# Blosc/c-blosc

Measured on NVIDIA H100. Metric: compress+decompress GB/s, higher is better.
Workload: dtype u8

## Files before the change

### c-blosc_b200/csrc/backend_cuda.cu

```cuda
#include <cuda_runtime.h>
#include <stdio.h>
#include <stdlib.h>

#include "b2_backend.h"
#include "dev_chunk.cuh"
#include "dev_filters.cuh"

struct b2_stream_s {
  cudaStream_t s;
};

#define B2_MAX_DEVICES 64
static int g_sms[B2_MAX_DEVICES];
static int g_prof_on = 0;
static double g_prof_ms[B2_K_COUNT];
static long long g_prof_n[B2_K_COUNT];
static long long g_launches = 0;

#define CK(call)                                                                              \
  do {                                                                                        \
    cudaError_t e_ = (call);                                                                  \
    if (e_ != cudaSuccess) {                                                                  \
      fprintf(stderr, "blosc_b200: CUDA error %s at %s:%d\n", cudaGetErrorString(e_), __FILE__, __LINE__); \
      return -1;                                                                              \
// ... 118 lines not shown
static void prof_resolve() {
  std::lock_guard<std::mutex> lk(g_prof_mu);
  for (auto& p : g_pending) {
    float ms = 0;
    cudaEventSynchronize(p.e1);
    cudaEventElapsedTime(&ms, p.e0, p.e1);
    g_prof_ms[p.kind] += ms; g_prof_n[p.kind]++;
    cudaEventDestroy(p.e0); cudaEventDestroy(p.e1);
  }
  g_pending.clear();
}

extern "C" void b2_prof_enable(int on) { g_prof_on = on; }
extern "C" void b2_prof_reset(void) { prof_resolve(); for (int i = 0; i < B2_K_COUNT; i++) { g_prof_ms[i] = 0; g_prof_n[i] = 0; } }
extern "C" int b2_prof_get(int kind, double* ms, long long* n) {
  if (kind < 0 || kind >= B2_K_COUNT) return -1;
  prof_resolve();
  if (ms) *ms = g_prof_ms[kind];
  if (n) *n = g_prof_n[kind];
  return 0;
}
extern "C" long long b2_launch_count(void) { return g_launches; }

extern "C" int b2_launch_filter(const FilterArgs* a, b2_stream_t s) {
  const bool bit = a->mode >= FILT_BITSHUFFLE;
  const bool inverse = a->mode == FILT_UNSHUFFLE || a->mode == FILT_BITUNSHUFFLE;
  const long long nblocks = (a->nbytes + a->blocksize - 1) / a->blocksize;
  const long long ipb = (a->blocksize / a->typesize + FILT_TILE - 1) / FILT_TILE + 1;
  long long ctas = (nblocks * ipb + FILT_WARPS - 1) / FILT_WARPS;
  void (*kern)(FilterArgs) = a->typesize == 2 ? filter_kernel<2> : a->typesize == 4 ? filter_kernel<4> : a->typesize == 8 ? filter_kernel<8> : filter_kernel<0>;
  const size_t smem = bit ? FILT_WARPS * 16 * FILT_TILE : 0;
  int per_sm = 0;
  if (cudaOccupancyMaxActiveBlocksPerMultiprocessor(&per_sm, kern, FILT_WARPS * 32, smem) != cudaSuccess || per_sm < 1) { cudaGetLastError(); per_sm = 4; }
  const long long cap = (long long)num_sms() * per_sm;
  if (ctas > cap) ctas = cap;
  if (ctas < 1) ctas = 1;
  ProfScope ps(inverse ? B2_K_UNFILTER : B2_K_FILTER, s->s);
  kern<<<(unsigned)ctas, FILT_WARPS * 32, smem, s->s>>>(*a);
  CK(cudaGetLastError());
  return 0;
}

static int team_wanted(const EncodeArgs* a) {
  static int env = -2;
  if (env == -2) { const char* e = getenv("BLOSC_B200_LZ4_TEAM"); env = (e && *e) ? (atoi(e) != 0) : -1; }
  if (a->codec != B2_CODEC_LZ4 || a->table_bytes != LZ4_TABLE_BYTES) return 0;
  return env >= 0 ? env : (a->map.nsplits == 4 && !a->many);
}

#ifdef B2_LZ4_CYCLES
extern "C" int b2_lz4_cycles_read(unsigned long long* dst, int nstreams) {
  if (nstreams > LZ4C_MAXSTREAMS) nstreams = LZ4C_MAXSTREAMS;
  CK(cudaDeviceSynchronize());
  CK(cudaMemcpyFromSymbol(dst, g_lz4_cycles, (size_t)nstreams * LZ4C_N * sizeof(unsigned long long)));
  return nstreams;
}
#endif

template <class Args>
static Args take_tickets(const Args* a, long long jobs, long long drawers) {
  Args args = *a;
  args.queue_base = *a->queue_base_host;
  *a->queue_base_host += (unsigned)jobs + (unsigned)drawers;
  return args;
}

extern "C" int b2_launch_encode(const EncodeArgs* a, b2_stream_t s) {
  if (team_wanted(a)) {
    int ctas = a->map.nstreams;
    const int cap = num_sms() * TEAM_CTAS_PER_SM;
    if (ctas > cap) ctas = cap;
    if (ctas <= 0) return 0;
    ProfScope ps(B2_K_ENCODE, s->s);
    EncodeArgs args = take_tickets(a, a->map.nstreams, ctas);
    args.num_sms = num_sms();
    encode_team_kernel<<<ctas, TEAM_WARPS * 32, TEAM_SMEM_BYTES, s->s>>>(args);
    CK(cudaGetLastError());
    return 0;
  }
  int wpc = 65536 / a->table_bytes;
  if (wpc > 4) wpc = 4;
  if (wpc < 1) wpc = 1;
  const int ctas = (a->map.nstreams + wpc - 1) / wpc;
  if (ctas <= 0) return 0;
  ProfScope ps(B2_K_ENCODE, s->s);
  encode_kernel<<<ctas, wpc * 32, (size_t)wpc * a->table_bytes, s->s>>>(take_tickets(a, a->map.nstreams, ctas * wpc));
  CK(cudaGetLastError());
  return 0;
}

extern "C" int b2_launch_fast(const FastArgs* a, b2_stream_t s) {
  if (a->map.nstreams <= 0) return 0;
  {
    int ctas = (a->map.nstreams + INDEX_WARPS - 1) / INDEX_WARPS;
    ProfScope ps(B2_K_INDEX, s->s);
    index_kernel<<<ctas, INDEX_WARPS * 32, INDEX_WARPS * FAST_TAB_BYTES, s->s>>>(*a);
    CK(cudaGetLastError());
  }
  {
    void (*parse)(FastArgs) = a->codec == B2_CODEC_LZ4 ? parse_kernel : a->codec == B2_CODEC_ZLIB ? dparse_kernel : zparse_kernel;
    const long long njobs = (long long)a->map.nfull * a->map.nsplits * a->groups_full + a->groups_left;
    const int threads = a->threads;
    const size_t smem = (size_t)a->win_bytes + 64;
    int per_sm = (int)((size_t)220 * 1024 / (smem + 1024));
    if (per_sm * threads > 2048) per_sm = 2048 / threads;
    if (per_sm < 1) per_sm = 1;
    long long ctas = njobs;
// ... 108 lines not shown
```

### c-blosc_b200/csrc/dev_chunk.cuh

```cuda
#pragma once
#include "b2_args.h"
#include "dev_blosclz.cuh"
#include "dev_common.cuh"
#include "dev_inflate.cuh"
#include "dev_lz4.cuh"
#include "dev_lz4fast.cuh"
#include "dev_lz4dpair.cuh"
#include "dev_zstd.cuh"
#include "dev_zstdenc.cuh"
#include "dev_deflate.cuh"
#include "dev_snappy.cuh"



DEV int next_stream(int* queue, unsigned base, const StreamMap& m) {
  int job = 0;
  if (lane_id() == 0) job = (int)((unsigned)atomicAdd(queue, 1) - base);
  job = __shfl_sync(FULLMASK, job, 0);
  if (job >= m.nstreams) return -1;
  const int nfs = m.nfull * m.nsplits;
  if (m.leftover) {
    if (job == 0) return nfs;
    job--;
  }
// ... 112 lines not shown
    if (lane_id() == 0) { a.csizes[idx] = c; a.needs[idx] = need; }
    mine++;
    __syncwarp();
  }
  return mine;
}

__global__ void encode_kernel(EncodeArgs a) {
#ifdef SIMT_EMU
  u8* smem = simt::g_dynsmem;
#else
  extern __shared__ __align__(16) u8 smem[];
#endif
  const int warp = (int)(threadIdx.x >> 5);
  void* tab = smem + (size_t)warp * a.table_bytes;
  const int mine = encode_streams(a, [&](int, const u8* in, int len, u8* out, int* need) {
    if (a.codec == B2_CODEC_LZ4) {
      if (a.table_bytes == LZ4_TAB17_BYTES) return lz4_encode_warp<false, true>(in, len, out, len, a.accel, tab, need);
      if (len < 65536 + LZ4_MFLIMIT - 1) return lz4_encode_warp<true>(in, len, out, len, a.accel, tab, need);
      return lz4_encode_warp<false>(in, len, out, len, a.accel, tab, need);
    }
    return blz_encode_warp(a.clevel, in, len, out, len, a.split_flag, tab, a.table_bytes, need);
  });
  streams_done(a.done, a.map.nstreams, mine, [&] { if (a.fold_scan) warp_scan_blocks(a.scan); });
}


#define TEAM_WARPS 4
#define TEAM_CTAS_PER_SM 8
#define TEAM_SMEM_BYTES (LZ4_TABLE_BYTES + ((LZ4T_SMEM_BYTES + 15) & ~15))
#define TEAM_SM_SLOTS 1024
#ifndef SIMT_EMU
__device__ unsigned g_team_sm_seq[TEAM_SM_SLOTS];
#endif
__global__ void __launch_bounds__(TEAM_WARPS * 32, TEAM_CTAS_PER_SM) encode_team_kernel(EncodeArgs a) {
#ifdef SIMT_EMU
  u8* smem = simt::g_dynsmem;
#else
  extern __shared__ __align__(16) u8 smem[];
#endif
  void* tab = smem;
  Lz4Team* tm = (Lz4Team*)(smem + LZ4_TABLE_BYTES);
  const int warp = (int)(threadIdx.x >> 5);
  int walker = (int)((blockIdx.x / (unsigned)(a.num_sms > 0 ? a.num_sms : 1)) & 3u);
#ifndef SIMT_EMU
  if (lane_id() == 0) { unsigned w; asm volatile("mov.u32 %0, %%warpid;" : "=r"(w)); tm->sub[warp] = (int)(w & 3u); }
  if (threadIdx.x == 0) {
    unsigned sm; asm volatile("mov.u32 %0, %%smid;" : "=r"(sm));
    tm->slot = (int)(atomicAdd(&g_team_sm_seq[sm % TEAM_SM_SLOTS], 1u) & 3u);
  }
#endif
  if (threadIdx.x == 0) { tm->cmd = 0; tm->gen = 0; }
#ifdef B2_LZ4_CYCLES
  if (threadIdx.x < LZ4C_N) tm->cyc[threadIdx.x] = 0;
#endif
  __syncthreads();
#ifndef SIMT_EMU
  for (int k = 3; k >= 0; k--) if (tm->sub[k] == tm->slot) walker = k;
#endif
  if (warp != walker) { lz4_team_preparer(tm, tab, (warp - walker - 1) & 3); return; }
  const int mine = encode_streams(a, [&](int idx, const u8* in, int len, u8* out, int* need) {
    LZ4C_T(c_total);
    const int c = len < 65536 + LZ4_MFLIMIT - 1 ? lz4_encode_warp<true, false, true>(in, len, out, len, a.accel, tab, need, tm)
                                                 : lz4_encode_warp<false, false, true>(in, len, out, len, a.accel, tab, need, tm);
#ifdef B2_LZ4_CYCLES
    {
      const unsigned long long total = (unsigned long long)(clock64() - c_total);
      unsigned smid, wid;
      asm volatile("mov.u32 %0, %%smid;" : "=r"(smid));
      asm volatile("mov.u32 %0, %%warpid;" : "=r"(wid));
      __syncwarp();
      const int k = lane_id();
      if (idx < LZ4C_MAXSTREAMS && k < LZ4C_N)
        g_lz4_cycles[idx][k] = k == LZ4C_TOTAL ? total : k == LZ4C_SMID ? smid : k == LZ4C_SUBP ? (wid & 3u) : tm->cyc[k];
      __syncwarp();
      if (k < LZ4C_N) tm->cyc[k] = 0;
    }
#endif
    return c;
  });
  if (lane_id() == 0) *(volatile int*)&tm->cmd = LZ4T_QUIT;
  __syncwarp();
  __threadfence_block();
  bar_arrive(LZ4T_BAR_GO(0), 64); bar_arrive(LZ4T_BAR_GO(1), 64); bar_arrive(LZ4T_BAR_GO(2), 64);
  streams_done(a.done, a.map.nstreams, mine, [&] { if (a.fold_scan) warp_scan_blocks(a.scan); });
}


#define INDEX_WARPS 4
__global__ void __launch_bounds__(INDEX_WARPS * 32) index_kernel(FastArgs a) {
#ifdef SIMT_EMU
  u8* smem = simt::g_dynsmem;
#else
  extern __shared__ __align__(16) u8 smem[];
#endif
  const int warp = (int)(threadIdx.x >> 5);
  u32* tab = (u32*)(smem + (size_t)warp * FAST_TAB_BYTES);
  for (int idx = (int)blockIdx.x * INDEX_WARPS + warp; idx < a.map.nstreams; idx += (int)gridDim.x * INDEX_WARPS) {
    int block, len, split;
    long long off;
    stream_locate(a.map, idx, &block, &off, &len, &split);
    lz4f_index_warp(a.in + off, len, a.prev + off, tab, (u32)a.hash_mask);
    __syncwarp();
  }
}

template <bool ZSTD, int MAXD = 65535>
DEV void fast_parse_body(const FastArgs& a, u8* smem) {
  u32* sdata = (u32*)smem;
  int* sjob = (int*)(smem + a.win_bytes + 48);
  const int tid = (int)threadIdx.x, lane = lane_id();
  const int nfs = a.map.nfull * a.map.nsplits;
  const int njobs = nfs * a.groups_full + a.groups_left;
  const int spw = a.win_bytes / FAST_SEG;
  for (;;) {
    if (tid == 0) { sjob[0] = (int)((unsigned)atomicAdd(a.queue, 1) - a.queue_base); sjob[1] = 0; }
    __syncthreads();
    const int job = sjob[0];
    if (job >= njobs) break;
    int idx, g, K;
    if (job < a.groups_left) { idx = nfs; g = job; K = a.segs_left; }
    else {
      const int j = job - a.groups_left;
      const int per_split = a.map.nfull * a.groups_full;
      const int s = j / per_split, r = j - s * per_split;
      const int b = r / a.groups_full;
      g = r - b * a.groups_full;
      idx = b * a.map.nsplits + s; K = a.segs_full;
    }
// ... 612 lines not shown
```

### c-blosc_b200/csrc/dev_lz4.cuh

```cuda
#pragma once
#include "dev_common.cuh"

#define LZ4_MFLIMIT 12
#define LZ4_LASTLITERALS 5
#define LZ4_TABLE_BYTES 16384
#define LZ4_TAB17_BYTES (8192 + 512)
#define LZ4_TAB17_MINLEN 65547
#define LZ4_TAB17_MAXLEN 131072

template <bool U16>
DEV u32 lz4_hash_at(const u8* __restrict__ s, int pos) {
  if (U16) return (ld_u32(s + pos) * 2654435761u) >> (32 - 13);
  const u64 seq = (u64)ld_u32(s + pos) | ((u64)s[pos + 4] << 32);
  return (u32)(((seq << 24) * 889523592379ull) >> (64 - 12));
}

#define LZ4_SCALAR_PROBES 4

DEV long long lz4_probe_offset(int it, int accel) {
  if (it == 0) return 0;
  const long long m = it - 1;
  const long long c = m >> 6;
  return 1 + m * accel + 32 * c * (c - 1) + c * (m - 64 * c);
}
// ... 104 lines not shown
#else
  const int q = p + sb.sal;
  const u32* w = sb.s32 + (q >> 2);
  return __funnelshift_r(__ldg(w), __ldg(w + 1), (u32)(q & 3) * 8u);
#endif
}

template <bool U16>
DEV u32 lz4_hash_seq(u32 lo, u32 b4) {
  if (U16) return (lo * 2654435761u) >> (32 - 13);
  const u64 seq = (u64)lo | ((u64)(b4 & 0xffu) << 32);
  return (u32)(((seq << 24) * 889523592379ull) >> (64 - 12));
}

DEV int lz4_count_tail(const StreamBase& sb, const u8* __restrict__ s, int p, int q, int limit, int n) {
  if (p + 136 <= n) {
    const int lane = lane_id();
    const u32 x = ldp_win4(sb, p + 4 * lane) ^ ldp_win4(sb, q + 4 * lane);
    const unsigned full = __ballot_sync(FULLMASK, x == 0u);
    if (full != FULLMASK) {
      const int fl = __ffs((int)~full) - 1;
      return fl * 4 + eq_bytes32(__shfl_sync(FULLMASK, x, fl));
    }
    return 128 + warp_count_match(s, p + 128, q + 128, limit);
  }
  return warp_count_match(s, p, q, limit);
}

DEV int lz4_catch_up(const u8* __restrict__ s, int ip, int match, int anchor, int back) {
  const int lane = lane_id();
  for (;;) {
    const int a = ip - 1 - back - lane, b = match - 1 - back - lane;
    const bool ok = a >= anchor && b >= 0 && s[a] == s[b];
    const unsigned m = __ballot_sync(FULLMASK, ok);
    const int step = m == FULLMASK ? 32 : __ffs((int)~m) - 1;
    back += step;
    if (step < 32) return back;
  }
}

#ifdef SIMT_EMU
static long long g_dbg_lz4t_sessions = 0, g_dbg_lz4t_seqs = 0, g_dbg_lz4t_stale = 0, g_dbg_lz4t_x[6];
enum {
  LZ4T_S_HIT0,
  LZ4T_S_STALE = 4,
  LZ4T_S_MISS4,
  LZ4T_S_LIT,
  LZ4T_S_CAPPED,
  LZ4T_S_LONG,
  LZ4T_S_HUGE,
  LZ4T_S_N
};
static long long g_dbg_lz4t_s[LZ4T_S_N];
#define LZ4T_DBG(x) do { if (lane_id() == 0) (x)++; } while (0)
#else
#define LZ4T_DBG(x) do {} while (0)
#endif
#ifndef LZ4T_TILES
#define LZ4T_TILES 12
#endif
#ifndef LZ4T_AHEAD
#define LZ4T_AHEAD 8
#endif
#ifndef LZ4T_NAP
#define LZ4T_NAP 128
#endif
#define LZ4T_RING (32 * LZ4T_TILES)
#define LZ4T_BAR_IDLE(i) (1 + (i))
#define LZ4T_BAR_GO(i) (4 + (i))
#define LZ4T_QUIT 1
#define LZ4T_STOP 0x7fffffff
#define LZ4T_END 0xffffffffu
#define LZ4T_LONG 13
#define LZ4T_HSHIFT 19
#define LZ4T_BACKCAP 7
static_assert(LZ4T_TILES % 3 == 0 && LZ4T_AHEAD >= 1 && LZ4T_AHEAD < LZ4T_TILES && LZ4T_RING > 15 + 255 + 4, "team ring layout");
#define LZ4T_PREFETCH 512

enum {
  LZ4C_TOTAL,
  LZ4C_START,
  LZ4C_SESSION,
  LZ4C_FULLWAIT,
  LZ4C_REPROBE,
  LZ4C_SEARCH,
  LZ4C_SESSIONS, LZ4C_SEQS, LZ4C_CHAIN_SEQS,
  LZ4C_PREP_BUSY,
  LZ4C_PREP_OWN,
  LZ4C_PREP_GATHER,
  LZ4C_PREP_TILES,
  LZ4C_SMID, LZ4C_SUBP,
  LZ4C_STALE,
  LZ4C_N = 16
};
#ifdef B2_LZ4_CYCLES
#define LZ4C_MAXSTREAMS 16384
__device__ unsigned long long g_lz4_cycles[LZ4C_MAXSTREAMS][LZ4C_N];
#define LZ4C_T(t) const long long t = clock64()
#define LZ4C_TW(t) const long long t = TEAM ? clock64() : 0ll
#define LZ4C_ADD(k, v) do { if (lane_id() == 0) atomicAdd(&tm->cyc[k], (unsigned long long)(v)); } while (0)
#define LZ4C_SPAN(k, t) LZ4C_ADD(k, clock64() - (t))
#else
#define LZ4C_T(t) do {} while (0)
#define LZ4C_TW(t) do {} while (0)
#define LZ4C_ADD(k, v) do {} while (0)
#define LZ4C_SPAN(k, t) do {} while (0)
#endif

struct Lz4Team {
  uint2 vd[LZ4T_RING];
  int rdy[LZ4T_TILES];
  const u8* s;
  int n;
  int u16;
  int wt;
  int gen;
  int cmd;
  int sub[4];
  int slot;
#ifdef B2_LZ4_CYCLES
  unsigned long long cyc[LZ4C_N];
#endif
};
#define LZ4T_SMEM_BYTES ((int)sizeof(Lz4Team))

DEV int lz4t_ld_i32(const int* p) { return *(const volatile int*)p; }
DEV void lz4t_st_i32(int* p, int v) { *(volatile int*)p = v; }

template <bool U16>
DEV void lz4_team_prepare_tile(Lz4Team* tm, const void* tabmem, const u8* s, int n, int tile) {
  const int lane = lane_id();
  const int w0 = 32 * tile, p = w0 + lane;
  const int e = (tile % LZ4T_TILES) * 32 + lane;
  if (w0 + 31 + 24 > n) { tm->vd[e] = make_uint2(0u, LZ4T_END); return; }
  const StreamBase sb = make_stream_base(s);
  u32 r[5], a0, a1, a2, a3, a4, c0, c1, c2, c3, c4;
  LZ4C_T(c_t0);
  ldp_raw20(sb, p, r);
  ldp_take17(sb, p, r, a0, a1, a2, a3, a4);
  const u32 h = lz4_hash_seq<U16>(a0, a1);
  const int snap = U16 ? (int)((const volatile u16*)tabmem)[h] : (int)((const volatile u32*)tabmem)[h];
  u32 vx = h << LZ4T_HSHIFT, sn = LZ4T_END;
  if ((unsigned)snap < (unsigned)p) {
    LZ4C_T(c_t1);
    LZ4C_ADD(LZ4C_PREP_OWN, c_t1 - c_t0);
    ldp_gather17(sb, snap, c0, c1, c2, c3, c4);
    const u32 x1 = a1 ^ c1, x2 = a2 ^ c2, x3 = a3 ^ c3;
    u32 m;
    if (x1) m = (u32)(__ffs((int)x1) - 1) >> 3;
    else if (x2) m = 4u + ((u32)(__ffs((int)x2) - 1) >> 3);
    else if (x3) m = 8u + ((u32)(__ffs((int)x3) - 1) >> 3);
    else m = a4 != c4 ? 12u : (u32)LZ4T_LONG;
    const bool hit = (U16 || snap + 65535 >= p) && c0 == a0;
    u32 bk = 0;
    if (hit) {
      if (snap >= 8) {
        u32 p0, p1, q0, q1;
        ldp_win8(sb, p - 8, p0, p1);
        ldp_win8(sb, snap - 8, q0, q1);
        const u32 y1 = p1 ^ q1, z0 = (u32)__clz((int)(p0 ^ q0)) >> 3;
        bk = y1 ? (u32)__clz((int)y1) >> 3 : 4u + (z0 < 3u ? z0 : 3u);
      } else {
        while (bk < (u32)snap && s[p - 1 - (int)bk] == s[snap - 1 - (int)bk]) bk++;
      }
    }
    vx |= (hit ? 1u : 0u) | (m << 2) | (bk << 8);
    sn = (u32)snap;
    LZ4C_SPAN(LZ4C_PREP_GATHER, c_t1);
  }
  tm->vd[e] = make_uint2(vx, sn);
}

DEV void lz4_team_preparer(Lz4Team* tm, const void* tabmem, int i) {
  for (;;) {
    bar_sync(LZ4T_BAR_GO(i), 64);
    if (lz4t_ld_i32(&tm->cmd) == LZ4T_QUIT) return;
    const u8* s = *(const u8* const volatile*)&tm->s;
    const int n = lz4t_ld_i32(&tm->n), u16 = lz4t_ld_i32(&tm->u16);
    for (int tile = i;; tile += 3) {
      int w;
      for (;;) {
        w = __shfl_sync(FULLMASK, lz4t_ld_i32(&tm->wt), 0);
        if (w == LZ4T_STOP) break;
        if (tile < w) tile = w + (i + 3 - w % 3) % 3;
        if (tile <= w + LZ4T_AHEAD) break;
        __nanosleep(LZ4T_NAP);
      }
      if (w == LZ4T_STOP) break;
      LZ4C_T(c_go);
      lz4d_prefetch(s, 32 * tile + LZ4T_PREFETCH + lane_id(), n);
      if (u16) lz4_team_prepare_tile<true>(tm, tabmem, s, n, tile);
      else lz4_team_prepare_tile<false>(tm, tabmem, s, n, tile);
      __syncwarp();
      if (lane_id() == 0) { __threadfence_block(); lz4t_st_i32(&tm->rdy[tile % LZ4T_TILES], tile + 1); }
      LZ4C_SPAN(LZ4C_PREP_BUSY, c_go);
      LZ4C_ADD(LZ4C_PREP_TILES, 1);
    }
    __syncwarp();
    bar_arrive(LZ4T_BAR_IDLE(i), 64);
  }
}

DEV void lz4t_reach(Lz4Team* tm, int ip, int& wt, int& vt) {
  const int lo = (ip - 2) >> 5, hi = ip >> 5;
  if (lo > wt + LZ4T_AHEAD) LZ4T_DBG(g_dbg_lz4t_x[2]);
  if (lo != wt) { wt = lo; lz4t_st_i32(&tm->wt, lo); }
  for (int t = vt + 1 > lo ? vt + 1 : lo; t <= hi; t++) {
    const int* r = &tm->rdy[t % LZ4T_TILES];
    if (lz4t_ld_i32(r) != t + 1) {
      LZ4T_DBG(g_dbg_lz4t_x[5]);
      do { __syncwarp(); } while (__any_sync(FULLMASK, lz4t_ld_i32(r) != t + 1));
    }
  }
  if (hi > vt) vt = hi;
}

template <bool U16>
DEV bool lz4t_search(Lz4Team* tm, smem_addr_t vda, void* tabmem, const StreamBase& sb, int n, int anchor, int accel,
                     int& twt, int& tvt, u32& pk, u32& snap, int& ip, bool& hit, int& match, int& back, int& lit,
                     bool& have_mc, int& mc_carry) {
  u16* tab16 = (u16*)tabmem;
  u32* tab32 = (u32*)tabmem;
  const int mfl1 = n - LZ4_MFLIMIT + 1;
  ip = anchor + 1;
  int it = 0, pos = ip;
  for (;; it++) {
    if (it == LZ4_SCALAR_PROBES) { LZ4T_DBG(g_dbg_lz4t_s[LZ4T_S_MISS4]); lit = it; return false; }
    pos = ip + (it ? 1 + (it - 1) * accel : 0);
    if (ip + 1 + it * accel > mfl1) { lit = it; return false; }
    if ((pos >> 5) > tvt) lz4t_reach(tm, pos, twt, tvt);
    u32 qk, qs;
    smem_ld_u32x2(vda, ((u32)pos % (u32)LZ4T_RING) << 3, qk, qs);
    const u32 h = qk >> LZ4T_HSHIFT;
    const int cand = U16 ? (int)tab16[h] : (int)tab32[h];
    __syncwarp();
    if (cand != (int)qs) { LZ4T_DBG(g_dbg_lz4t_s[LZ4T_S_STALE]); lit = it; return false; }
    if (U16) tab16[h] = (u16)pos; else tab32[h] = (u32)pos;
    if (qk & 1u) { pk = qk; snap = qs; break; }
  }
  LZ4T_DBG(g_dbg_lz4t_s[LZ4T_S_HIT0 + it]);
  const int vb = (int)((pk >> 8) & 7u), dist = pos - anchor;
  const int bq = vb < dist ? vb : dist;
  int m = (int)((pk >> 2) & 15u);
  if (m == LZ4T_LONG) {
    LZ4T_DBG(g_dbg_lz4t_s[LZ4T_S_LONG]);
    m = LZ4T_LONG + lz4_count_tail(sb, sb.s, pos + 4 + LZ4T_LONG, (int)snap + 4 + LZ4T_LONG, n - LZ4_LASTLITERALS, n);
  }
  if (bq == dist && bq + m < 15 + 255) {
    const int mc = bq + m;
    snap -= (u32)bq;
    pk = 1u | ((u32)(mc < LZ4T_LONG ? mc : LZ4T_LONG) << 2);
    ip = anchor;
    LZ4C_ADD(LZ4C_SEQS, 1);
    LZ4C_ADD(LZ4C_CHAIN_SEQS, ~0ull);
    return true;
  }
  hit = true; ip = pos; match = (int)snap;
  have_mc = true; mc_carry = m;
  back = bq;
  if (vb == LZ4T_BACKCAP && dist > LZ4T_BACKCAP) {
    LZ4T_DBG(g_dbg_lz4t_s[LZ4T_S_CAPPED]);
    back = lz4_catch_up(sb.s, pos, (int)snap, anchor, LZ4T_BACKCAP);
  } else if (bq != dist) LZ4T_DBG(g_dbg_lz4t_s[LZ4T_S_LIT]);
  else LZ4T_DBG(g_dbg_lz4t_s[LZ4T_S_HUGE]);
  lit = pos - back - anchor;
  return false;
}

template <bool U16, bool PACK, bool TEAM>
DEV int lz4_encode_stream(const u8* __restrict__ s, const int n, u8* __restrict__ d, const int cap,
                          const int accel, void* tabmem, int* need_out, Lz4Team* tm) {
  const int lane = lane_id();
  const StreamBase sb = make_stream_base(s);
  u16* tab16 = (u16*)tabmem;
  u32* tab32 = (u32*)tabmem;
  u32* tabhi = (u32*)((u8*)tabmem + 8192);
#define LZ4_TGET(h) (U16 ? (int)tab16[h] : PACK ? ((int)tab16[h] | (int)(((tabhi[(h) >> 5] >> ((h) & 31u)) & 1u) << 16)) : (int)tab32[h])
#define LZ4_TPUT(h, v) do { if (U16) tab16[h] = (u16)(v); else if (PACK) { tab16[h] = (u16)(v); const u32 m_ = 1u << ((h) & 31u); \
                            if ((v) & 0x10000) atomicOr(&tabhi[(h) >> 5], m_); else atomicAnd(&tabhi[(h) >> 5], ~m_); } \
                            else tab32[h] = (u32)(v); } while (0)

  for (int i = lane; i < (PACK ? LZ4_TAB17_BYTES : LZ4_TABLE_BYTES) / 4; i += 32) tab32[i] = 0;
  __syncwarp();

  const bool limited = (long long)cap < (long long)n + n / 255 + 16;
  const int olimit = cap;
  const int mfl1 = n - LZ4_MFLIMIT + 1;
  const int matchlimit = n - LZ4_LASTLITERALS;
  int ip = 1, anchor = 0, op = 0;
  int need = 0;
#define LZ4_LIMIT(v) do { const int v_ = (v); if (v_ > need) need = v_; if (limited && v_ > olimit) return 0; } while (0)

  int w0 = -(1 << 30);
  u32 wq0 = 0, wq1 = 0, wq2 = 0, wh = 0;
  int pb = -(1 << 30);
  u32 pq0 = 0, pq1 = 0, pq2 = 0, pq3 = 0;
  int nrec = 0, recop = 0;
  u32 rec = 0;
  int twt = 0, tvt = -1;
#define LZ4_FLUSH_CHECKED() do { if (nrec) { LZ4_LIMIT(op + (1 + LZ4_LASTLITERALS)); } LZ4_FLUSH(); } while (0)
#define LZ4_FLUSH() do { if (lane < nrec) { d[recop] = (u8)rec; d[recop + 1] = (u8)(rec >> 8); d[recop + 2] = (u8)(rec >> 16); \
                                             if ((rec & 15u) == 15u) d[recop + 3] = (u8)(rec >> 24); } nrec = 0; } while (0)

  if (n >= LZ4_MFLIMIT + 1) {
    bool post = false;
    for (;;) {
      int match = 0, lit = 0, back = 0;
      u32 ipn = 0, cn = 0;
      bool have_next = false, hit = false, imm = false, have_mc = false;
      int mc_carry = 0;

      bool scalar_post = post;
      if (TEAM && post && ip + 64 <= n) {
        scalar_post = false;
        bool finished = false;
        if (nrec >= 24) LZ4_FLUSH_CHECKED();
        LZ4T_DBG(g_dbg_lz4t_sessions);
        LZ4C_T(c_s0);
        LZ4C_ADD(LZ4C_SESSIONS, 1);
        if ((ip - 2) >> 5 <= twt + LZ4T_AHEAD) LZ4T_DBG(g_dbg_lz4t_x[3]);
        lz4t_reach(tm, ip, twt, tvt);
        __syncwarp();
        LZ4C_SPAN(LZ4C_START, c_s0);
        LZ4C_T(c_s1);
        const smem_addr_t vda = smem_addr(tm->vd);
        u32 e = (u32)ip % (u32)LZ4T_RING;
        for (;;) {
          u32 pk, snap;
          smem_ld_u32x2(vda, e << 3, pk, snap);
          const u32 h2 = smem_ld_u32(vda, (e >= 2u ? e - 2u : e - 2u + LZ4T_RING) << 3) >> LZ4T_HSHIFT;
          const u32 h = pk >> LZ4T_HSHIFT;
          LZ4_TPUT(h2, ip - 2);
          const int cand = LZ4_TGET(h);
          __syncwarp();
          if (cand != (int)snap) {
            LZ4T_DBG(g_dbg_lz4t_stale); LZ4C_ADD(LZ4C_STALE, 1);
            scalar_post = true; break;
          }
          LZ4_TPUT(h, ip);
          if (!(pk & 1u)) {
            LZ4T_DBG(g_dbg_lz4t_x[4]);
            if constexpr (TEAM) {
              if (!lz4t_search<U16>(tm, vda, tabmem, sb, n, anchor, accel, twt, tvt, pk, snap, ip, hit, match, back, lit, have_mc, mc_carry))
                break;
              if (nrec >= 24) LZ4_FLUSH_CHECKED();
            } else { ip++; break; }
          }
          const int off = ip - (int)snap;
          int mc = (int)((pk >> 2) & 15u);
          if (mc == LZ4T_LONG) {
            LZ4T_DBG(g_dbg_lz4t_x[0]);
            mc = LZ4T_LONG + lz4_count_tail(sb, s, ip + 4 + LZ4T_LONG, ip - off + 4 + LZ4T_LONG, matchlimit, n);
            if (mc >= 15 + 255) {
              hit = true; imm = true; match = ip - off;
              have_mc = true; mc_carry = mc;
              LZ4T_DBG(g_dbg_lz4t_x[1]);
              break;
            }
          }
          const bool ext = mc >= 15;
          LZ4T_DBG(g_dbg_lz4t_seqs);
          LZ4C_ADD(LZ4C_CHAIN_SEQS, 1);
          if (lane == nrec) { rec = (ext ? 15u | ((u32)(mc - 15) << 24) : (u32)mc) | ((u32)off << 8); recop = op; }
          nrec++;
          op += ext ? 4 : 3;
          ip += mc + 4;
          e += (u32)(mc + 4);
          if (e >= (u32)LZ4T_RING) e -= (u32)LZ4T_RING;
          anchor = ip;
          if (ip + 64 > n) {
            if (ip >= mfl1) finished = true;
            else scalar_post = true;
            break;
          }
          if ((ip >> 5) > tvt) {
            LZ4C_T(c_w);
            lz4t_reach(tm, ip, twt, tvt);
            LZ4C_SPAN(LZ4C_FULLWAIT, c_w);
            if (nrec >= 24) LZ4_FLUSH_CHECKED();
          }
        }
        LZ4C_SPAN(LZ4C_SESSION, c_s1);
        if (finished) break;
      }
      if (!TEAM && post && ip + 64 <= n) {
        scalar_post = false;
        bool room = true;
        for (;;) {
          if (ip - 2 < w0 || ip > w0 + 31) {
            if (nrec >= 24) LZ4_FLUSH_CHECKED();
            if (ip - 2 >= pb && ip <= pb + 31) { w0 = pb; ldp_take12(sb, w0 + lane, pq0, pq1, pq2, pq3, wq0, wq1, wq2); }
            else { w0 = ip - 2; ldp_win12(sb, w0 + lane, wq0, wq1, wq2); }
            wh = lz4_hash_seq<U16>(wq0, wq1);
            pb = w0 + 30;
            if (pb + 31 + 16 <= n) ldp_raw12(sb, pb + lane, pq0, pq1, pq2, pq3);
            else pb = -(1 << 30);
            lz4d_prefetch(s, w0 + 192, lane == 0 ? n : 0);
          }
          const int li = ip - w0;
          const u32 h2 = __shfl_sync(FULLMASK, wh, li - 2);
          const u32 h = __shfl_sync(FULLMASK, wh, li);
          const u32 seq = __shfl_sync(FULLMASK, wq0, li);
          const u32 n4 = __shfl_sync(FULLMASK, wq1, li);
          const u32 n8 = __shfl_sync(FULLMASK, wq2, li);
          if (lane == 0) LZ4_TPUT(h2, ip - 2);
          __syncwarp();
          const int cand = LZ4_TGET(h);
          __syncwarp();
          if (lane == 0) LZ4_TPUT(h, ip);
          u32 c0, c1, c2;
          ldp_win12(sb, cand, c0, c1, c2);
          if (!((U16 || cand + 65535 >= ip) && c0 == seq)) { ip++; break; }
          int mc;
          const u32 x1 = n4 ^ c1, x2 = n8 ^ c2;
          if (x1 | x2) {
            const u32 xx = x1 ? x1 : x2;
            mc = ((__ffs((int)xx) - 1) >> 3) + (x1 ? 0 : 4);
          } else {
            u32 p3, p4, q3, q4;
            ldp_win8(sb, ip + 12, p3, p4);
            ldp_win8(sb, cand + 12, q3, q4);
            const u32 x3 = p3 ^ q3, x4 = p4 ^ q4;
            if (x3) mc = 8 + eq_bytes32(x3);
            else if (x4) mc = 12 + eq_bytes32(x4);
            else mc = 16 + lz4_count_tail(sb, s, ip + 20, cand + 20, matchlimit, n);
          }
          if (mc >= 15 + 255) {
            hit = true; imm = true; match = cand;
            have_mc = true; mc_carry = mc;
            break;
          }
          const bool ext = mc >= 15;
          const int off = ip - cand;
// ... 147 lines not shown
          warp_fill_bytes(d + op, nff, 255);
          if (lane == 0) d[op + nff] = (u8)(len - nff * 255);
          op += nff + 1;
        } else tokval = (u32)lit << 4;
        warp_copy_bytes(d + op, s + anchor, lit);
        op += lit;
        if (lane == 0) { d[op] = (u8)off; d[op + 1] = (u8)(off >> 8); }
        op += 2;
        LZ4_LIMIT(op + (1 + LZ4_LASTLITERALS) + (mc + 240) / 255);
        if (mc >= 15) {
          tokval += 15;
          const int rest = mc - 15, nff = rest / 255;
          warp_fill_bytes(d + op, nff, 255);
          if (lane == 0) d[op + nff] = (u8)(rest - nff * 255);
          op += nff + 1;
        } else tokval += (u32)mc;
        if (lane == 0) d[token] = (u8)tokval;
      }

      anchor = ip;
      if (ip >= mfl1) break;
      post = true;
    }
  }

  LZ4_FLUSH_CHECKED();
  const int lastRun = n - anchor;
  LZ4_LIMIT(op + lastRun + 1 + (lastRun + 255 - 15) / 255);
  if (lastRun >= 15) {
    const int acc = lastRun - 15, nff = acc / 255;
    if (lane == 0) d[op] = (u8)(15u << 4);
    op++;
    warp_fill_bytes(d + op, nff, 255);
    if (lane == 0) d[op + nff] = (u8)(acc - nff * 255);
    op += nff + 1;
  } else {
    if (lane == 0) d[op] = (u8)(lastRun << 4);
    op++;
  }
  warp_copy_bytes(d + op, s + anchor, lastRun);
  op += lastRun;
  *need_out = need;
  return op;
#undef LZ4_FLUSH_CHECKED
#undef LZ4_FLUSH
#undef LZ4_LIMIT
#undef LZ4_TGET
#undef LZ4_TPUT
}

DEV void lz4t_begin(Lz4Team* tm, const u8* s, int n, bool u16) {
  const int lane = lane_id();
  for (int i = lane; i < LZ4T_TILES; i += 32) tm->rdy[i] = 0;
  if (lane == 0) { tm->s = s; tm->n = n; tm->u16 = u16 ? 1 : 0; tm->wt = 0; tm->gen = tm->gen + 1; }
  __syncwarp();
  __threadfence_block();
  bar_arrive(LZ4T_BAR_GO(0), 64); bar_arrive(LZ4T_BAR_GO(1), 64); bar_arrive(LZ4T_BAR_GO(2), 64);
}
DEV void lz4t_end(Lz4Team* tm) {
  __syncwarp();
  if (lane_id() == 0) lz4t_st_i32(&tm->wt, LZ4T_STOP);
  __syncwarp();
  bar_sync(LZ4T_BAR_IDLE(0), 64); bar_sync(LZ4T_BAR_IDLE(1), 64); bar_sync(LZ4T_BAR_IDLE(2), 64);
}

template <bool U16, bool PACK = false, bool TEAM = false>
DEV int lz4_encode_warp(const u8* __restrict__ s, const int n, u8* __restrict__ d, const int cap,
                        const int accel, void* tabmem, int* need_out, Lz4Team* tm = nullptr) {
  if (TEAM) lz4t_begin(tm, s, n, U16);
  const int c = lz4_encode_stream<U16, PACK, TEAM>(s, n, d, cap, accel, tabmem, need_out, tm);
  if (TEAM) lz4t_end(tm);
  return c;
}

enum {
  LZ4D_H_DENSE_SHIFT = 0,
  LZ4D_H_DENSE_LONGCAP = 9,
  LZ4D_H_DENSE_BAD,
  LZ4D_H_DENSE_BAD0,
  LZ4D_H_DENSE_FEW,
  LZ4D_H_DENSE_RING, LZ4D_H_DENSE_GLOBAL,
  LZ4D_H_LONE_RING, LZ4D_H_LONE_GLOBAL, LZ4D_H_LONE_PERIOD,
  LZ4D_H_BATCH_FAST, LZ4D_H_BATCH_WALK,
  LZ4D_H_BATCH_RING, LZ4D_H_BATCH_GLOBAL,
  LZ4D_H_SINGLE_RING, LZ4D_H_SINGLE_GLOBAL,
  LZ4D_H_GEN_LITBUMP,
  LZ4D_H_GEN_OFF0, LZ4D_H_GEN_RING, LZ4D_H_GEN_GLOBAL, LZ4D_H_GEN_LONG, LZ4D_H_GEN_LAST,
  LZ4D_NHIT
};
#ifdef SIMT_EMU
static long long g_dbg_lz4d_batch_seqs = 0, g_dbg_lz4d_fast_seqs = 0, g_dbg_lz4d_general_seqs = 0, g_dbg_lz4d_dense_seqs = 0;
#define LZ4D_DBG(x) do { if (lane == 0) (x)++; } while (0)
#define LZ4D_DBGN(x, n) do { if (lane == 0) (x) += (n); } while (0)
static int g_lz4d_fail_line = 0;
#define LZ4D_FAIL (g_lz4d_fail_line = g_lz4d_fail_line ? g_lz4d_fail_line : __LINE__, -1)
static long long g_lz4d_hit[LZ4D_NHIT];
#define LZ4D_HIT(id) do { if (lane == 0) g_lz4d_hit[id]++; } while (0)
#define LZ4D_HITL(id, c) do { if (c) g_lz4d_hit[id]++; } while (0)
#else
#define LZ4D_DBG(x) do {} while (0)
#define LZ4D_DBGN(x, n) do {} while (0)
#define LZ4D_FAIL (-1)
#define LZ4D_HIT(id) do {} while (0)
#define LZ4D_HITL(id, c) do {} while (0)
#endif
#define LZ4D_RING 16384
// ... 377 lines not shown
```

Measured before the change: 121.7.

## Batch team LZ4 sequence chain into warp-parallel windows of hash updates

Replaces the one-sequence-at-a-time walker loop in the team LZ4 encoder with a window scheme. Up to 16 precomputed sequences are gathered per window, and their hash table reads and writes run in parallel across lanes, two lanes per sequence. Duplicate hash keys are handled with a shared-memory seen-bitmap and match_any, and the first stale candidate truncates the window. The aim is to cut the serial per-sequence latency on the walker warp. The cost is extra shared memory (a 1 KB bitmap), atomics and shuffles per window, plus wasted work when windows are cut short.

```diff
diff --git a/c-blosc_b200/csrc/backend_cuda.cu b/c-blosc_b200/csrc/backend_cuda.cu
--- a/c-blosc_b200/csrc/backend_cuda.cu
+++ b/c-blosc_b200/csrc/backend_cuda.cu
@@ -194,7 +194,7 @@
 extern "C" int b2_lz4_cycles_read(unsigned long long* dst, int nstreams) {
   if (nstreams > LZ4C_MAXSTREAMS) nstreams = LZ4C_MAXSTREAMS;
   CK(cudaDeviceSynchronize());
-  CK(cudaMemcpyFromSymbol(dst, g_lz4_cycles, (size_t)nstreams * LZ4C_N * sizeof(unsigned long long)));
+  CK(cudaMemcpyFromSymbol(dst, g_lz4_cycles, (size_t)nstreams * LZ4C_NREC * sizeof(unsigned long long)));
   return nstreams;
 }
 #endif
diff --git a/c-blosc_b200/csrc/dev_chunk.cuh b/c-blosc_b200/csrc/dev_chunk.cuh
--- a/c-blosc_b200/csrc/dev_chunk.cuh
+++ b/c-blosc_b200/csrc/dev_chunk.cuh
@@ -188,7 +188,7 @@
 #endif
   if (threadIdx.x == 0) { tm->cmd = 0; tm->gen = 0; }
 #ifdef B2_LZ4_CYCLES
-  if (threadIdx.x < LZ4C_N) tm->cyc[threadIdx.x] = 0;
+  if (threadIdx.x < LZ4C_NREC) tm->cyc[threadIdx.x] = 0;
 #endif
   __syncthreads();
 #ifndef SIMT_EMU
@@ -207,10 +207,10 @@
       asm volatile("mov.u32 %0, %%warpid;" : "=r"(wid));
       __syncwarp();
       const int k = lane_id();
-      if (idx < LZ4C_MAXSTREAMS && k < LZ4C_N)
+      if (idx < LZ4C_MAXSTREAMS && k < LZ4C_NREC)
         g_lz4_cycles[idx][k] = k == LZ4C_TOTAL ? total : k == LZ4C_SMID ? smid : k == LZ4C_SUBP ? (wid & 3u) : tm->cyc[k];
       __syncwarp();
-      if (k < LZ4C_N) tm->cyc[k] = 0;
+      if (k < LZ4C_NREC) tm->cyc[k] = 0;
     }
 #endif
     return c;
diff --git a/c-blosc_b200/csrc/dev_lz4.cuh b/c-blosc_b200/csrc/dev_lz4.cuh
--- a/c-blosc_b200/csrc/dev_lz4.cuh
+++ b/c-blosc_b200/csrc/dev_lz4.cuh
@@ -180,9 +180,25 @@
   LZ4T_S_N
 };
 static long long g_dbg_lz4t_s[LZ4T_S_N];
+enum {
+  LZ4T_W_WINDOWS,
+  LZ4T_W_ELEMS,
+  LZ4T_W_STALE0, LZ4T_W_STALEJ,
+  LZ4T_W_FWD,
+  LZ4T_W_CROSS,
+  LZ4T_W_MISS0, LZ4T_W_MISSJ,
+  LZ4T_W_LONG0, LZ4T_W_LONGJ,
+  LZ4T_W_HUGE,
+  LZ4T_W_END, LZ4T_W_CAP, LZ4T_W_TILE,
+  LZ4T_W_FULL,
+  LZ4T_W_N
+};
+static long long g_dbg_lz4t_w[LZ4T_W_N];
 #define LZ4T_DBG(x) do { if (lane_id() == 0) (x)++; } while (0)
+#define LZ4T_DBGN(x, v) do { if (lane_id() == 0) (x) += (v); } while (0)
 #else
 #define LZ4T_DBG(x) do {} while (0)
+#define LZ4T_DBGN(x, v) do {} while (0)
 #endif
 #ifndef LZ4T_TILES
 #define LZ4T_TILES 12
@@ -202,7 +218,9 @@
 #define LZ4T_LONG 13
 #define LZ4T_HSHIFT 19
 #define LZ4T_BACKCAP 7
+#define LZ4T_W 16
 static_assert(LZ4T_TILES % 3 == 0 && LZ4T_AHEAD >= 1 && LZ4T_AHEAD < LZ4T_TILES && LZ4T_RING > 15 + 255 + 4, "team ring layout");
+static_assert(2 * LZ4T_W <= 32, "window layout");
 #define LZ4T_PREFETCH 512
 
 enum {
@@ -221,9 +239,13 @@
   LZ4C_STALE,
   LZ4C_N = 16
 };
+enum {
+  LZ4C_WINDOWS = LZ4C_N, LZ4C_W_STALE, LZ4C_W_MISS, LZ4C_W_LONG, LZ4C_W_END, LZ4C_W_CAP, LZ4C_W_TILE,
+  LZ4C_NREC
+};
 #ifdef B2_LZ4_CYCLES
 #define LZ4C_MAXSTREAMS 16384
-__device__ unsigned long long g_lz4_cycles[LZ4C_MAXSTREAMS][LZ4C_N];
+__device__ unsigned long long g_lz4_cycles[LZ4C_MAXSTREAMS][LZ4C_NREC];
 #define LZ4C_T(t) const long long t = clock64()
 #define LZ4C_TW(t) const long long t = TEAM ? clock64() : 0ll
 #define LZ4C_ADD(k, v) do { if (lane_id() == 0) atomicAdd(&tm->cyc[k], (unsigned long long)(v)); } while (0)
@@ -246,8 +268,9 @@
   int cmd;
   int sub[4];
   int slot;
+  u32 seen[8192 / 32];
 #ifdef B2_LZ4_CYCLES
-  unsigned long long cyc[LZ4C_N];
+  unsigned long long cyc[LZ4C_NREC];
 #endif
 };
 #define LZ4T_SMEM_BYTES ((int)sizeof(Lz4Team))
@@ -343,6 +366,12 @@
   if (hi > vt) vt = hi;
 }
 
+DEV void lz4t_extend(Lz4Team* tm, int wt, int& vt) {
+  const int t = vt + 1 + lane_id();
+  const bool ready = t <= wt + LZ4T_AHEAD && lz4t_ld_i32(&tm->rdy[t % LZ4T_TILES]) == t + 1;
+  vt += __ffs((int)~__ballot_sync(FULLMASK, ready)) - 1;
+}
+
 template <bool U16>
 DEV bool lz4t_search(Lz4Team* tm, smem_addr_t vda, void* tabmem, const StreamBase& sb, int n, int anchor, int accel,
                      int& twt, int& tvt, u32& pk, u32& snap, int& ip, bool& hit, int& match, int& back, int& lit,
@@ -439,10 +468,9 @@
       int mc_carry = 0;
 
       bool scalar_post = post;
-      if (TEAM && post && ip + 64 <= n) {
+      if constexpr (TEAM) if (post && ip + 64 <= n) {
         scalar_post = false;
         bool finished = false;
-        if (nrec >= 24) LZ4_FLUSH_CHECKED();
         LZ4T_DBG(g_dbg_lz4t_sessions);
         LZ4C_T(c_s0);
         LZ4C_ADD(LZ4C_SESSIONS, 1);
@@ -453,60 +481,139 @@
         LZ4C_T(c_s1);
         const smem_addr_t vda = smem_addr(tm->vd);
         u32 e = (u32)ip % (u32)LZ4T_RING;
+        bool given = false;
+        u32 gpk = 0, gsnap = 0;
         for (;;) {
-          u32 pk, snap;
-          smem_ld_u32x2(vda, e << 3, pk, snap);
-          const u32 h2 = smem_ld_u32(vda, (e >= 2u ? e - 2u : e - 2u + LZ4T_RING) << 3) >> LZ4T_HSHIFT;
-          const u32 h = pk >> LZ4T_HSHIFT;
-          LZ4_TPUT(h2, ip - 2);
-          const int cand = LZ4_TGET(h);
+          if (nrec > 32 - LZ4T_W) {
+#ifdef SIMT_EMU
+            if (limited && op + 1 + LZ4_LASTLITERALS > olimit) LZ4T_DBG(g_dbg_lz4t_w[LZ4T_W_FULL]);
+#endif
+            LZ4_FLUSH_CHECKED();
+          }
+          lz4t_extend(tm, twt, tvt);
+          int cnt = 0, q = ip, why;
+          u32 ee = e, pk, snap;
+          if (given) { pk = gpk; snap = gsnap; } else smem_ld_u32x2(vda, ee << 3, pk, snap);
+          int jq = 0;
+          u32 je = 0, jpk = 0, jsnap = 0;
+          for (;;) {
+            if (lane == cnt) { jq = q; je = ee; jpk = pk; jsnap = snap; }
+            cnt++;
+            const u32 step = ((pk >> 2) & 15u) + 4u;
+            u32 en = ee + step;
+            if (en >= (u32)LZ4T_RING) en -= (u32)LZ4T_RING;
+            u32 npk, nsnap;
+            smem_ld_u32x2(vda, en << 3, npk, nsnap);
+            if (!(pk & 1u)) { why = LZ4C_W_MISS; break; }
+            if (step == LZ4T_LONG + 4u) { why = LZ4C_W_LONG; break; }
+            q += (int)step; ee = en;
+            if (cnt == LZ4T_W) { why = LZ4C_W_CAP; break; }
+            if (q + 64 > n) { why = LZ4C_W_END; break; }
+            if ((q >> 5) > tvt) { why = LZ4C_W_TILE; break; }
+            pk = npk; snap = nsnap;
+          }
+          u32 jh2 = 0;
+          if (lane < cnt) jh2 = smem_ld_u32(vda, (je >= 2u ? je - 2u : je - 2u + LZ4T_RING) << 3) >> LZ4T_HSHIFT;
+          const int el = lane >> 1;
+          const bool odd = (lane & 1) != 0;
+          const u32 sh2 = __shfl_sync(FULLMASK, jh2, el), sh = __shfl_sync(FULLMASK, jpk >> LZ4T_HSHIFT, el);
+          const int sq = __shfl_sync(FULLMASK, jq, el);
+          const u32 ssnap = __shfl_sync(FULLMASK, jsnap, el);
+          const bool act = lane < 2 * cnt && !(given && lane < 2);
+          const u32 skey = odd ? sh : sh2;
+          const int spos = odd ? sq : sq - 2;
+          int look = 0;
+          bool dup = false;
+          if (act) {
+            if (odd) look = LZ4_TGET(skey);
+            const u32 bit = 1u << (skey & 31u);
+            dup = (atomicOr(&tm->seen[skey >> 5], bit) & bit) != 0;
+          }
+          unsigned peers = 1u << lane;
+          if (__ballot_sync(FULLMASK, dup)) {
+            peers = __match_any_sync(FULLMASK, act ? skey : 0x80000000u | (u32)lane);
+            const unsigned lower = peers & ((1u << lane) - 1u);
+            const int fpos = __shfl_sync(FULLMASK, spos, lower ? 31 - __clz((int)lower) : lane);
+            if (act && odd && lower) look = fpos;
+#ifdef SIMT_EMU
+            const unsigned fwd = __ballot_sync(FULLMASK, act && odd && lower != 0);
+            const unsigned cross = __ballot_sync(FULLMASK, act && !odd && ((peers & 0xaaaaaaaau) & ~(2u << lane)) != 0);
+            if (fwd) LZ4T_DBG(g_dbg_lz4t_w[LZ4T_W_FWD]);
+            if (cross) LZ4T_DBG(g_dbg_lz4t_w[LZ4T_W_CROSS]);
+#endif
+          }
+          const unsigned bad = __ballot_sync(FULLMASK, act && odd && look != (int)ssnap);
+          const int nv = bad ? (__ffs((int)bad) - 1) >> 1 : cnt;
+          LZ4T_DBG(g_dbg_lz4t_w[LZ4T_W_WINDOWS]);
+          LZ4T_DBGN(g_dbg_lz4t_w[LZ4T_W_ELEMS], nv);
           __syncwarp();
-          if (cand != (int)snap) {
-            LZ4T_DBG(g_dbg_lz4t_stale); LZ4C_ADD(LZ4C_STALE, 1);
+          const unsigned le = nv >= 16 ? FULLMASK : (1u << (2 * nv)) - 1u;
+          if (act && lane < 2 * nv && (((peers & le) >> lane) >> 1) == 0) LZ4_TPUT(skey, spos);
+          if (act) tm->seen[skey >> 5] = 0u;
+          __syncwarp();
+          const int nb = nv < cnt || why == LZ4C_W_MISS || why == LZ4C_W_LONG ? (nv < cnt ? nv : cnt - 1) : cnt;
+          const u32 rv = (u32)((jpk >> 2) & 15u) | ((u32)(jq - (int)jsnap) << 8);
+          const u32 rmine = __shfl_sync(FULLMASK, rv, (lane - nrec) & 31);
+          if (lane >= nrec && lane < nrec + nb) { rec = rmine; recop = op + 3 * (lane - nrec); }
+          nrec += nb;
+          op += 3 * nb;
+          LZ4T_DBGN(g_dbg_lz4t_seqs, nb);
+          LZ4C_ADD(LZ4C_CHAIN_SEQS, nb);
+          LZ4C_ADD(LZ4C_WINDOWS, 1);
+          if (nb < cnt) {
+            ip = __shfl_sync(FULLMASK, jq, nb);
+            e = __shfl_sync(FULLMASK, je, nb);
+            snap = __shfl_sync(FULLMASK, jsnap, nb);
+          } else { ip = q; e = ee; }
+          anchor = ip;
+          given = false;
+          if (nv < cnt) {
+            LZ4T_DBG(g_dbg_lz4t_stale); LZ4C_ADD(LZ4C_STALE, 1); LZ4C_ADD(LZ4C_W_STALE, 1);
+            LZ4T_DBG(g_dbg_lz4t_w[nv ? LZ4T_W_STALEJ : LZ4T_W_STALE0]);
             scalar_post = true; break;
           }
-          LZ4_TPUT(h, ip);
-          if (!(pk & 1u)) {
+          LZ4C_ADD(why, 1);
+          if (why == LZ4C_W_MISS) {
             LZ4T_DBG(g_dbg_lz4t_x[4]);
-            if constexpr (TEAM) {
-              if (!lz4t_search<U16>(tm, vda, tabmem, sb, n, anchor, accel, twt, tvt, pk, snap, ip, hit, match, back, lit, have_mc, mc_carry))
-                break;
-              if (nrec >= 24) LZ4_FLUSH_CHECKED();
-            } else { ip++; break; }
+            LZ4T_DBG(g_dbg_lz4t_w[nb ? LZ4T_W_MISSJ : LZ4T_W_MISS0]);
+            if (!lz4t_search<U16>(tm, vda, tabmem, sb, n, anchor, accel, twt, tvt, gpk, gsnap, ip, hit, match, back, lit, have_mc, mc_carry))
+              break;
+            given = true;
+            continue;
           }
-          const int off = ip - (int)snap;
-          int mc = (int)((pk >> 2) & 15u);
-          if (mc == LZ4T_LONG) {
+          if (why == LZ4C_W_LONG) {
             LZ4T_DBG(g_dbg_lz4t_x[0]);
-            mc = LZ4T_LONG + lz4_count_tail(sb, s, ip + 4 + LZ4T_LONG, ip - off + 4 + LZ4T_LONG, matchlimit, n);
+            LZ4T_DBG(g_dbg_lz4t_w[nb ? LZ4T_W_LONGJ : LZ4T_W_LONG0]);
+            const int off = ip - (int)snap;
+            const int mc = LZ4T_LONG + lz4_count_tail(sb, s, ip + 4 + LZ4T_LONG, ip - off + 4 + LZ4T_LONG, matchlimit, n);
             if (mc >= 15 + 255) {
               hit = true; imm = true; match = ip - off;
               have_mc = true; mc_carry = mc;
               LZ4T_DBG(g_dbg_lz4t_x[1]);
+              LZ4T_DBG(g_dbg_lz4t_w[LZ4T_W_HUGE]);
               break;
             }
-          }
-          const bool ext = mc >= 15;
-          LZ4T_DBG(g_dbg_lz4t_seqs);
-          LZ4C_ADD(LZ4C_CHAIN_SEQS, 1);
-          if (lane == nrec) { rec = (ext ? 15u | ((u32)(mc - 15) << 24) : (u32)mc) | ((u32)off << 8); recop = op; }
-          nrec++;
-          op += ext ? 4 : 3;
-          ip += mc + 4;
-          e += (u32)(mc + 4);
-          if (e >= (u32)LZ4T_RING) e -= (u32)LZ4T_RING;
-          anchor = ip;
+            const bool ext = mc >= 15;
+            LZ4T_DBG(g_dbg_lz4t_seqs);
+            LZ4C_ADD(LZ4C_CHAIN_SEQS, 1);
+            if (lane == nrec) { rec = (ext ? 15u | ((u32)(mc - 15) << 24) : (u32)mc) | ((u32)off << 8); recop = op; }
+            nrec++;
+            op += ext ? 4 : 3;
+            ip += mc + 4;
+            e += (u32)(mc + 4);
+            if (e >= (u32)LZ4T_RING) e -= (u32)LZ4T_RING;
+            anchor = ip;
+          } else if (why == LZ4C_W_CAP) LZ4T_DBG(g_dbg_lz4t_w[LZ4T_W_CAP]);
+          else if (why == LZ4C_W_TILE) LZ4T_DBG(g_dbg_lz4t_w[LZ4T_W_TILE]);
           if (ip + 64 > n) {
+            if (why == LZ4C_W_END) LZ4T_DBG(g_dbg_lz4t_w[LZ4T_W_END]);
             if (ip >= mfl1) finished = true;
             else scalar_post = true;
             break;
           }
-          if ((ip >> 5) > tvt) {
-            LZ4C_T(c_w);
-            lz4t_reach(tm, ip, twt, tvt);
-            LZ4C_SPAN(LZ4C_FULLWAIT, c_w);
-            if (nrec >= 24) LZ4_FLUSH_CHECKED();
-          }
+          LZ4C_T(c_w);
+          lz4t_reach(tm, ip, twt, tvt);
+          LZ4C_SPAN(LZ4C_FULLWAIT, c_w);
         }
         LZ4C_SPAN(LZ4C_SESSION, c_s1);
         if (finished) break;
@@ -760,6 +867,7 @@
 DEV void lz4t_begin(Lz4Team* tm, const u8* s, int n, bool u16) {
   const int lane = lane_id();
   for (int i = lane; i < LZ4T_TILES; i += 32) tm->rdy[i] = 0;
+  for (int i = lane; i < 8192 / 32; i += 32) tm->seen[i] = 0;
   if (lane == 0) { tm->s = s; tm->n = n; tm->u16 = u16 ? 1 : 0; tm->wt = 0; tm->gen = tm->gen + 1; }
   __syncwarp();
   __threadfence_block();
```

Measured after the change: 128.1 (median of 6 runs). 5.3% higher.
